# EnricoMiccoli/nodal

Hardware: AMD Instinct MI355X
Metric: circuits_per_sec (higher is better)
Workload: dtype f64; 1 GPU; cfg3: grid(1000) 1e6 nodes, sparse CSR path; n=999999, nnz=4995995, parallelism=one GPU

## Files before the change

nodal_amd/csrc/sagg.hip:

```cpp
#include <hip/hip_ext.h>

#include <atomic>
#include <type_traits>

#include "group.h"

int grounded_flags(nodal_ctx *h, uint8_t *flags_dev);

namespace {

using grp::TB;
constexpr int PW = 4;
constexpr int ACAP = 64;
constexpr int RCAP = 96;
constexpr int RCAP_SMALL = 512;
constexpr int RCAP_SMALL_ROWS = 16384;
inline int rcap_for(int64_t nc) { return nc <= RCAP_SMALL_ROWS ? RCAP_SMALL : RCAP; }
constexpr int W0_MAX = 32;
constexpr int COARSEST = 64;
constexpr int MAX_LEVELS = 12;
constexpr int MIS_ROUNDS = 6;
constexpr int TAIL_MAX_N = 1024;
constexpr int TAIL_LEVELS = 6;
constexpr int TAIL_LDS_BUDGET = 150 * 1024;
// ... 72 lines not shown
    int nlev;
    TailLevelDesc lv[TAIL_LEVELS];
    const double *inv;
    int nu;
    int image_bytes;
    int lds_bytes;
    int skip;
    int slots;
    long long *stamps;
};

struct SHierarchy {
    std::vector<SLevel *> pool;
    int nlev = 0;
    int tail = -1;
    bool ready = false;
    bool kcycle = true;
    bool kfrozen = false;
    int kslot = -1, kcount = 0, ksamples = 0;
    int klevels = 1;
    int nu[3] = {2, 1, 2};
    bool dense_coarsest = true;
    DevBuf tail_stamps, tail_image, apcol, apval, aplen, bstat;
    DevBuf mvec;
    hipEvent_t ev_copy = nullptr;
    hipStream_t aux = nullptr;
    hipEvent_t ev_fork = nullptr, ev_join = nullptr, ev_flags = nullptr;
    bool aux_pending = false;
    bool aux_tried = false;
    bool want_flags = false;
    int flags_levels = 0;
    DevBuf stats, coarse_inv, mis_t, mis_m, mis_flag, mis_id, agg1, keys, rstart, cursor, lists;
    TailDesc td;
    uint64_t *host_stats = nullptr;
    bool sym_valid = false;
    uint64_t sym_epoch = 0;
    int64_t sym_n = 0, sym_nnz = 0;
    bool sym_general = false, sym_check = false;
    int32_t sym_floating = 0;
    hipGraph_t it_graph = nullptr;
    hipGraphExec_t it_exec = nullptr;
    uint64_t it_key = 0;
    bool refreshed = false;
    int last_iters = 0;
    int hint_iters = 0;
    int64_t hint_n = 0, hint_nnz = 0;
// ... 5 lines not shown
        return pool[l];
    }
    void drop_graph() {
        if (it_exec) (void)hipGraphExecDestroy(it_exec);
        if (it_graph) (void)hipGraphDestroy(it_graph);
        it_exec = nullptr;
        it_graph = nullptr;
        it_key = 0;
    }
    ~SHierarchy() {
        drop_graph();
        if (ev_copy) (void)hipEventDestroy(ev_copy);
        if (ev_fork) (void)hipEventDestroy(ev_fork);
        if (ev_join) (void)hipEventDestroy(ev_join);
        if (ev_flags) (void)hipEventDestroy(ev_flags);
        if (aux) (void)hipStreamDestroy(aux);
        for (SLevel *l : pool) {
            DevBuf *b[] = {&l->acol, &l->aval, &l->alen, &l->dinv, &l->agg, &l->pcol, &l->pval, &l->rcol,
                           &l->rval, &l->rlen, &l->vec, &l->part, &l->gflag, &l->avalf, &l->pvalf, &l->rvalf, &l->adcol};
            for (DevBuf *x : b) x->release();
            delete l;
        }
        tail_image.release();
        mvec.release();
        tail_stamps.release();
        bstat.release();
        apcol.release();
        apval.release();
        aplen.release();
        DevBuf *b[] = {&stats, &coarse_inv, &mis_t, &mis_m, &mis_flag, &mis_id, &agg1, &keys, &rstart, &cursor, &lists};
        for (DevBuf *x : b) x->release();
        if (host_stats) (void)hipHostFree(host_stats);
    }
};


constexpr int BSTAT_MAX = 65536;
__global__ __launch_bounds__(1024) void reduce_bstat(int nblocks, const uint32_t *__restrict__ bstat,
                                                     unsigned long long *__restrict__ stats, int slot_max,
                                                     int slot_sum) {
    __shared__ unsigned int s_max;
    __shared__ unsigned long long s_sum;
    if (threadIdx.x == 0) { s_max = 0; s_sum = 0; }
    __syncthreads();
    unsigned int m = 0;
    unsigned long long t = 0;
// ... 1088 lines not shown
        NODAL_HIP_TRY(h, hipEventRecord(H->ev_join, H->aux));
        if (H->want_flags && H->flags_levels == l) {
            if (l == 0) NODAL_TRY(grounded_flags(h, L->gflag.as<uint8_t>()));
            NODAL_HIP_TRY(h, hipMemsetAsync(C->gflag.p, 0, ((size_t)C->n + 63) & ~(size_t)63, st));
            flags_up<<<grid_for(n), TB, 0, st>>>(n, L->agg.as<int32_t>(), L->gflag.as<uint8_t>(), C->gflag.as<uint8_t>());
            NODAL_HIP_TRY(h, hipGetLastError());
            NODAL_HIP_TRY(h, hipEventRecord(H->ev_flags, H->aux));
            H->flags_levels = l + 1;
        }
        h->stream = main_st;
        st = main_st;
    }
    NODAL_TRY(galerkin_product<false>(h, H, l, forked ? H->ev_join : nullptr, forked ? 2 : 0));
    if (forked && H->flags_levels != l + 1) H->aux_pending = false;
    return NODAL_OK;
}

const void *tail_kernel(int slots) {
    return slots <= 8 ? reinterpret_cast<const void *>(k_tail<8>)
                      : slots <= 16 ? reinterpret_cast<const void *>(k_tail<16>)
                                    : reinterpret_cast<const void *>(k_tail<32>);
}

int build_tail(nodal_ctx *h, SHierarchy *H, const unsigned long long *hs) {
    H->tail = -1;
    const int last = H->nlev - 1;
    auto up16 = [](int x) { return (x + 15) & ~15; };
    for (int t = 1; t <= last; ++t) {
        if (H->pool[t]->n > TAIL_MAX_N || last - t + 1 > TAIL_LEVELS) continue;
        TailDesc d;
        memset(&d, 0, sizeof d);
        d.nlev = last - t + 1;
        d.nu = getenv("NODAL_SA_TAIL_NU") ? atoi(getenv("NODAL_SA_TAIL_NU")) : 3;
        if (d.nu < 1) d.nu = 1;
        int off = 0;
        for (int k = 0; k < d.nlev; ++k) {
            const SLevel *L = H->pool[t + k];
            TailLevelDesc &q = d.lv[k];
            q.n = (int)L->n; q.nc = (int)L->nc; q.ld = (int)L->ld; q.rld = (int)L->rld; q.width = L->maxlen;
            q.acol = L->acol.as<int32_t>(); q.aval = L->aval.as<double>();
            q.dinv = L->dinv.as<double>(); q.alen = L->alen.as<int32_t>();
            q.pcol = L->pcol.as<int32_t>(); q.pval = L->pval.as<double>();
            q.rcol = L->rcol.as<int32_t>(); q.rval = L->rval.as<double>(); q.rlen = L->rlen.as<int32_t>();
            if (k == d.nlev - 1) {
                q.o_aval = off; off = up16(off + (H->dense_coarsest ? q.n * q.n : q.n) * 8);
                continue;
            }
            const int maxr = (int)hs[(size_t)(t + k) * ST_COUNT + ST_MAXR];
// ... 14 lines not shown
            q.o_B = off; off = up16(off + q.n * 8);
            q.o_X = off; off = up16(off + q.n * 8);
            if (k == d.nlev - 1) continue;
            q.o_Y = off; off = up16(off + q.n * 8);
            q.o_R = off; off = up16(off + q.n * 8);
        }
        d.inv = H->dense_coarsest ? H->coarse_inv.as<double>() : nullptr;
        d.skip = d.nlev > 1 ? d.lv[0].o_dinv : 0;
        d.lds_bytes = off - d.skip;
        if (getenv("NODAL_TAIL_PROBE")) {
            NODAL_HIP_TRY(h, H->tail_stamps.reserve(64 * sizeof(long long)));
            d.stamps = H->tail_stamps.as<long long>();
        }
        if (d.lds_bytes > TAIL_LDS_BUDGET) continue;
        d.slots = d.nlev > 1 ? (d.lv[0].width + d.lv[0].lpr - 1) / d.lv[0].lpr : 1;
        if (d.slots > 32) continue;
        {
            static std::atomic<bool> lds_allowed[64][3];
            const int dev = h->device >= 0 && h->device < 64 ? h->device : 0;
            const int which = d.slots <= 8 ? 0 : (d.slots <= 16 ? 1 : 2);
            if (!lds_allowed[dev][which].load(std::memory_order_acquire)) {
                NODAL_HIP_TRY(h, hipFuncSetAttribute(tail_kernel(d.slots), hipFuncAttributeMaxDynamicSharedMemorySize,
                                                     TAIL_LDS_BUDGET));
                lds_allowed[dev][which].store(true, std::memory_order_release);
            }
        }
        NODAL_HIP_TRY(h, H->tail_image.reserve((size_t)d.image_bytes + 256));
        k_tail_pack<<<1, 1024, 0, h->stream>>>(d, H->tail_image.as<char>());
        NODAL_HIP_TRY(h, hipGetLastError());
        H->td = d;
        H->tail = t;
        break;
    }
    return NODAL_OK;
}

int sagg_refresh(nodal_ctx *h, SHierarchy *H, const int32_t *indptr0, const int32_t *indices0, const double *data0,
                 bool general, bool *ok) {
    *ok = false;
    hipStream_t st = h->stream;
    unsigned long long *dstats = H->stats.as<unsigned long long>();
    unsigned long long *hs = reinterpret_cast<unsigned long long *>(H->host_stats);
    NODAL_HIP_TRY(h, hipMemsetAsync(dstats, 0, (size_t)MAX_LEVELS * ST_COUNT * 8, st));
    SLevel *L0 = H->pool[0];
    const int64_t n0 = L0->n;
    {
        const unsigned gr = grid_for(n0);
        static const double spread = getenv("NODAL_SA_SPREAD") ? atof(getenv("NODAL_SA_SPREAD")) : 16.0;
        static const double share = getenv("NODAL_SA_SHARE") ? atof(getenv("NODAL_SA_SHARE")) : 0.9;
        row_stats<<<gr, TB, 0, st>>>(n0, indptr0, indices0, data0, share, spread, general, dstats, H->bstat.as<uint32_t>());
        reduce_bstat<<<1, 1024, 0, st>>>((int)gr, H->bstat.as<uint32_t>(), dstats, ST_MAXLEN, ST_GRADED);
    }
    csr_to_ell<<<grid_for(n0), TB, 0, st>>>(n0, L0->ld, indptr0, indices0, data0, L0->acol.as<int32_t>(),
                                           L0->aval.as<double>(), L0->avalf.as<float>(),
// ... 9 lines not shown
        const bool forked = H->aux != nullptr && nodal_extra_streams_ok(h) &&
                            !(getenv("NODAL_SA_FORK") && atoi(getenv("NODAL_SA_FORK")) == 0);
        hipStream_t rst = st;
        if (forked) {
            NODAL_HIP_TRY(h, hipEventRecord(H->ev_fork, st));
            NODAL_HIP_TRY(h, hipStreamWaitEvent(H->aux, H->ev_fork, 0));
            H->aux_pending = true;
            NODAL_TRY(galerkin_product<true>(h, H, l, nullptr, 1));
            rst = H->aux;
        }
        r_refresh<<<grid_for(C->n * 8), TB, 0, rst>>>(C->n, L->rld, L->rlen.as<int32_t>(), L->rcol.as<int32_t>(), L->ld,
                                                     L->pcol.as<int32_t>(), L->pval.as<double>(), L->rval.as<double>(),
                                                     L->rvalf.as<float>());
        NODAL_HIP_TRY(h, hipGetLastError());
        if (forked) NODAL_HIP_TRY(h, hipEventRecord(H->ev_join, H->aux));
        NODAL_TRY(galerkin_product<true>(h, H, l, forked ? H->ev_join : nullptr, forked ? 2 : 0));
        if (forked) H->aux_pending = false;
    }
    const int last = H->nlev - 1;
    if (H->dense_coarsest)
        coarsest_inverse<<<1, 256, 0, st>>>(H->pool[last]->A(), H->coarse_inv.as<double>(), dstats + (size_t)last * ST_COUNT);
    if (H->tail >= 0) k_tail_pack<<<1, 1024, 0, st>>>(H->td, H->tail_image.as<char>());
    NODAL_HIP_TRY(h, hipGetLastError());
    NODAL_HIP_TRY(h, hipMemcpyAsync(hs, dstats, (size_t)MAX_LEVELS * ST_COUNT * 8, hipMemcpyDeviceToHost, st));
    NODAL_WAIT_STREAM(h, st);
    const int64_t bar = n0 / 100 < 32 ? (n0 / 100 > 0 ? n0 / 100 : 1) : 32;
    if (hs[ST_BADDIAG] || (int64_t)hs[ST_GRADED] >= bar) return NODAL_OK;
    for (int k = 1; k < H->nlev; ++k)
        if (hs[(size_t)k * ST_COUNT + ST_BADDIAG] || hs[(size_t)k * ST_COUNT + ST_OVERFLOW]) return NODAL_OK;
    *ok = true;
    return NODAL_OK;
}

}

void sagg_destroy(nodal_ctx *h) {
    delete static_cast<SHierarchy *>(h->sagg);
    h->sagg = nullptr;
}

static int sagg_setup_csr_body(nodal_ctx *h, int64_t n0, int64_t nnz0, const int32_t *indptr0, const int32_t *indices0,
                               const double *data0, bool general, bool check_floating, bool *accepted, int32_t *floating);

int sagg_setup_csr(nodal_ctx *h, int64_t n0, int64_t nnz0, const int32_t *indptr0, const int32_t *indices0,
                   const double *data0, bool general, bool check_floating, bool *accepted, int32_t *floating) {
    const int s = sagg_setup_csr_body(h, n0, nnz0, indptr0, indices0, data0, general, check_floating, accepted, floating);
// ... 192 lines not shown
    *accepted = true;
    H->sym_valid = true;
    H->sym_epoch = h->struct_epoch;
    H->sym_n = n0;
    H->sym_nnz = nnz0;
    H->sym_general = general;
    H->sym_check = check_floating;
    H->sym_floating = *floating;
    memcpy(H->sym_stats, hs, sizeof H->sym_stats);
    return NODAL_OK;
}

int sagg_setup(nodal_ctx *h, bool *accepted, int32_t *floating) {
    return sagg_setup_csr(h, h->n, h->nnz, h->indptr.as<int32_t>(), h->indices.as<int32_t>(), h->data.as<double>(),
                          false, true, accepted, floating);
}

namespace {

int last_level(nodal_ctx *h, SHierarchy *H, int l, const double *b, double *out) {
    hipStream_t st = h->stream;
    SLevel *L = H->pool[l];
    const int64_t n = L->n;
    if (l == H->tail) {
        if (H->td.slots <= 8) k_tail<8><<<1, 1024, (size_t)H->td.lds_bytes, st>>>(H->td, H->tail_image.as<char>(), b, out, 1);
        else if (H->td.slots <= 16) k_tail<16><<<1, 1024, (size_t)H->td.lds_bytes, st>>>(H->td, H->tail_image.as<char>(), b, out, 1);
        else k_tail<32><<<1, 1024, (size_t)H->td.lds_bytes, st>>>(H->td, H->tail_image.as<char>(), b, out, 1);
    } else {
        k_coarsest<<<grid_for(n), TB, 0, st>>>(n, H->dense_coarsest ? H->coarse_inv.as<double>() : nullptr,
                                               L->dinv.as<double>(), b, out);
    }
    NODAL_HIP_TRY(h, hipGetLastError());
    return NODAL_OK;
}

void kcycle_schedule(SHierarchy *H, int it) {
    static const bool on = !(getenv("NODAL_SA_KFREEZE") && atoi(getenv("NODAL_SA_KFREEZE")) == 0);
    H->kfrozen = false;
    H->kslot = -1;
    if (!on || it < 0) return;
    if (it == 0) H->ksamples = 0;
    const bool adaptive = it < 4 || (it & 3) == 0;
    if (!adaptive && H->ksamples > 0) {
        H->kfrozen = true;
    } else if (it >= 2) {
        H->kslot = H->ksamples % 3;
        ++H->ksamples;
        H->kcount = H->ksamples < 3 ? H->ksamples : 3;
    }
}

template <typename TBV, typename TOUT>
int cycle(nodal_ctx *h, SHierarchy *H, int l, const TBV *b, const cyc_t *x0, TOUT *out, const SolveBufs *sb) {
    hipStream_t st = h->stream;
// ... 255 lines not shown
            return NODAL_OK;
        }
        f_direction<<<sb.g0, TB, 0, st>>>(sb.z, sb.p, sb.part_rz, sb.part_zap, sb.part_rr, sb.g0, sb.sc, it & 1, n);
        const unsigned tb0 = H->pool[0]->wfix ? TB : TB * LPR_RAGGED;
        if (timed) {
            SAGG_DISPATCH_W(H->pool[0]->wfix, (hipExtLaunchKernelGGL((f_spmv<W>), dim3(sb.g0), dim3(tb0), 0, st, e0, e1, 0,
                                                                     A0, (const double *)sb.p, sb.Ap, sb.part_pap,
                                                                     (const double *)sb.sc, it & 1)));
        } else {
            SAGG_DISPATCH_W(H->pool[0]->wfix, (f_spmv<W><<<sb.g0, tb0, 0, st>>>(A0, sb.p, sb.Ap, sb.part_pap, sb.sc, it & 1)));
        }
        f_update<<<sb.g0, TB, 0, st>>>(x, sb.r, sb.p, sb.Ap, sb.part_pap, sb.g0, dinv0, sb.x0, sb.part_rr, sb.sc, it & 1, n);
        NODAL_HIP_TRY(h, hipGetLastError());
        return NODAL_OK;
    };
    static const bool graphs = getenv("NODAL_SA_GRAPH") && atoi(getenv("NODAL_SA_GRAPH")) != 0;
    if (graphs && (H->refreshed || !do_setup)) {
        uint64_t key = 1469598103934665603ull;
        auto mix = [&](uint64_t v) { key = (key ^ v) * 1099511628211ull; };
        mix((uint64_t)(uintptr_t)base); mix((uint64_t)(uintptr_t)x); mix((uint64_t)n); mix((uint64_t)sb.g0);
        mix((uint64_t)H->nlev); mix((uint64_t)(H->tail + 1)); mix((uint64_t)H->kcycle); mix((uint64_t)H->klevels);
        mix((uint64_t)(H->nu[0] * 100 + H->nu[1] * 10 + H->nu[2])); mix((uint64_t)H->td.lds_bytes);
        mix((uint64_t)(uintptr_t)H->tail_image.p); mix((uint64_t)(uintptr_t)H->coarse_inv.p);
        for (int k = 0; k < H->nlev; ++k) {
            const SLevel *L = H->pool[k];
            const void *ps[] = {L->acol.p, L->aval.p, L->avalf.p, L->alen.p, L->dinv.p, L->pcol.p, L->pvalf.p,
                                L->rcol.p, L->rvalf.p, L->rlen.p, L->vec.p, L->part.p};
            for (const void *q : ps) mix((uint64_t)(uintptr_t)q);
            mix((uint64_t)L->n); mix((uint64_t)L->ld); mix((uint64_t)L->wfix); mix((uint64_t)L->rld);
        }
        if (H->it_exec && H->it_key != key) H->drop_graph();
        if (!H->it_exec) {
            hipGraph_t g = nullptr;
            hipGraphExec_t ex = nullptr;
            if (hipStreamBeginCapture(st, hipStreamCaptureModeThreadLocal) == hipSuccess) {
                int cs = iteration(0, false);
                if (cs == NODAL_OK) cs = iteration(1, false);
                const hipError_t ce = hipStreamEndCapture(st, &g);
                if (cs == NODAL_OK && ce == hipSuccess && g && hipGraphInstantiate(&ex, g, nullptr, nullptr, 0) == hipSuccess) {
                    H->it_graph = g;
                    H->it_exec = ex;
                    H->it_key = key;
                } else {
                    if (g) (void)hipGraphDestroy(g);
                    (void)hipGetLastError();
                }
// ... 54 lines not shown
            const double target = tol * tol * hs[F_BB];
            const double rr_ref = rr_prev > 0.0 ? rr_prev : hs[F_BB];
            const int64_t it_ref = rr_prev > 0.0 ? it_prev : 0;
            if (hs[F_RR] > 0.0 && hs[F_RR] < rr_ref && enqueued > it_ref) {
                const double rate = log(hs[F_RR] / rr_ref) / (double)(enqueued - it_ref);
                static const double look = getenv("NODAL_FCG_LOOK") ? atof(getenv("NODAL_FCG_LOOK")) : 0.75;
                next = (int)floor(look * log(target / hs[F_RR]) / rate);
            }
            if (next > enqueued) next = (int)enqueued;
            batch = next < 1 ? 1 : (next > 32 ? 32 : next);
            rr_prev = hs[F_RR];
            it_prev = enqueued;
        }
    }
    const int64_t its = status == 1 ? (int64_t)hs[F_ITERS] : enqueued;
    *iters = (int32_t)its;
    *resid = hs[F_BB] > 0 ? sqrt(hs[F_RR] / hs[F_BB]) : 0.0;
    const SLevel *L0 = H->pool[0];
    h->kern_alg = 12.0 * (double)L0->nnz + 4.0 * (double)n + 16.0 * (double)n;
    if (fuse_dir) h->kern_alg += 12.0 * (double)n;
    if (trace)
        fprintf(stderr, "[sagg] %d iterations (%lld enqueued, %d polls), relative residual %.2e, status %d\n", *iters,
                (long long)enqueued, polls, *resid, status);
    if (trace && H->tail >= 0 && H->td.stamps) {
        long long ts[64];
        if (hipMemcpy(ts, H->td.stamps, sizeof ts, hipMemcpyDeviceToHost) == hipSuccess) {
            fprintf(stderr, "[sagg] tail phases (us):");
            for (int k = 1; k < (int)ts[63] && k < 63; ++k) fprintf(stderr, " %.2f", (double)(ts[k] - ts[k - 1]) * 0.01);
            fprintf(stderr, "  total %.2f, image %d B, lds %d B\n", (double)(ts[ts[63] - 1] - ts[0]) * 0.01,
                    H->td.image_bytes, H->td.lds_bytes);
            for (int k = 0; k < H->td.nlev; ++k)
                fprintf(stderr, "[sagg]   tail level %d: n %d width %d lpr %d nq %d\n", k, H->td.lv[k].n,
                        H->td.lv[k].width, H->td.lv[k].lpr, H->td.lv[k].nq);
        }
    }
    if (status != 1) {
        H->last_iters = 0;
        return -1;
    }
    H->last_iters = (int)its;
    H->hint_iters = (int)its;
    H->hint_n = n;
    H->hint_nnz = H->pool[0]->nnz;
    *info = 0;
    return NODAL_OK;
}

// ... 2 lines not shown
```

nodal_amd/csrc/sagg_cycle.h:

```cpp
#pragma once

namespace {

constexpr int LPR_RAGGED = 1;
template <int W> struct RowLanes { static constexpr int value = W == 0 ? LPR_RAGGED : 1; };

template <class VT, class XF>
__device__ __forceinline__ double ell_row_lanes(const Ell &A, const VT *__restrict__ val, int64_t i, int sub, XF xf) {
    constexpr int Q = 8;
    const int32_t len = A.len[i];
    double acc = 0.0;
    for (int32_t s0 = sub; s0 < len; s0 += LPR_RAGGED * Q) {
        int32_t c[Q];
        double v[Q];
        if (A.dcol) {
#pragma unroll
            for (int q = 0; q < Q; ++q) {
                const bool ok = s0 + q * LPR_RAGGED < len;
                const int64_t at = (int64_t)(ok ? s0 + q * LPR_RAGGED : s0) * A.ld + i;
                c[q] = (int32_t)i + (int32_t)A.dcol[at];
                const VT loaded = val[at];
                v[q] = ok ? (double)loaded : 0.0;
            }
        } else {
// ... 423 lines not shown
        copy_u16(u16(L.o_pcol), L.pcol, L.n, L.ld, PW);
        copy_f64(f64(L.o_rval), L.rval, L.nc * RL, (int64_t)L.rld * RL, L.nq);
        copy_u16(u16(L.o_rcol), L.rcol, L.nc * RL, (int64_t)L.rld * RL, L.nq);
    }
    const TailLevelDesc &L = d.lv[last];
    if (d.inv) copy_f64(f64(L.o_aval), d.inv, L.n * L.n, L.n * L.n, 1);
    else copy_f64(f64(L.o_aval), L.dinv, L.n, L.n, 1);
}

template <int SLOTS>
__device__ __forceinline__ double reg_row(const double (&v)[SLOTS], const uint32_t (&c)[SLOTS / 2], int lpr,
                                          const double *x) {
    double s0 = 0.0, s1 = 0.0;
#pragma unroll
    for (int j = 0; j < SLOTS; j += 2) {
        s0 = fma(v[j], x[c[j / 2] & 0xffffu], s0);
        s1 = fma(v[j + 1], x[c[j / 2] >> 16], s1);
    }
    double s = s0 + s1;
    for (int off = lpr >> 1; off > 0; off >>= 1) s += __shfl_xor(s, off, 64);
    return s;
}

template <int SLOTS>
__global__ __launch_bounds__(1024) void k_tail(TailDesc d, const char *__restrict__ image,
                                               const double *__restrict__ rc, double *__restrict__ out, int vs) {
    extern __shared__ __attribute__((aligned(16))) char smem[];
    const int tid = threadIdx.x;
    const int voff = vs > 1 ? (int)blockIdx.x : 0;
    const int last = d.nlev - 1;
    const int TAIL_NU = d.nu;
    auto f64 = [&](int off) { return reinterpret_cast<double *>(smem + (off - d.skip)); };
    auto u16 = [&](int off) { return reinterpret_cast<uint16_t *>(smem + (off - d.skip)); };
    int stamp_no = 0;
    auto stamp = [&]() {
        if (d.stamps && tid == 0) d.stamps[stamp_no] = wall_clock64();
        ++stamp_no;
    };
    stamp();
    double v0[SLOTS];
    uint32_t c0[SLOTS / 2];
    {
        const TailLevelDesc &L = d.lv[0];
        const double *aval = reinterpret_cast<const double *>(image + L.o_aval);
        const uint16_t *acol = reinterpret_cast<const uint16_t *>(image + L.o_acol);
        const int lpr = L.lpr, sub = tid & (lpr - 1), i = tid / lpr, ii = i < L.n ? i : L.n - 1;
        const bool row = last > 0 && i < L.n;
#pragma unroll
        for (int j = 0; j < SLOTS; j += 2) {
            const int ta = sub + j * lpr, tb = ta + lpr;
            const bool ha = row && ta < L.width, hb = row && tb < L.width;
            const int ea = ha ? ta * L.n + ii : 0, eb = hb ? tb * L.n + ii : 0;
            const double va = aval[ea], vb = aval[eb];
            const uint32_t ca = acol[ea], cb = acol[eb];
            v0[j] = ha ? va : 0.0;
            v0[j + 1] = hb ? vb : 0.0;
            c0[j / 2] = (ha ? ca : 0u) | ((hb ? cb : 0u) << 16);
        }
    }
    {
        constexpr int FLY = (TAIL_LDS_BUDGET / 16 + 1023) / 1024;
        const int4 *src = reinterpret_cast<const int4 *>(image + d.skip);
        int4 *dst = reinterpret_cast<int4 *>(smem);
        const int pieces = (d.image_bytes - d.skip) / 16;
        int4 v[FLY];
#pragma unroll
        for (int u = 0; u < FLY; ++u) v[u] = src[tid + u * 1024 < pieces ? tid + u * 1024 : 0];
#pragma unroll
        for (int u = 0; u < FLY; ++u)
            if (tid + u * 1024 < pieces) dst[tid + u * 1024] = v[u];
    }
    for (int i = tid; i < d.lv[0].n; i += 1024) f64(d.lv[0].o_B)[i] = rc[(int64_t)i * vs + voff];
    __syncthreads();
    stamp();
    for (int k = 0; k < last; ++k) {
        const TailLevelDesc &L = d.lv[k];
        const double *aval = f64(L.o_aval), *dinv = f64(L.o_dinv), *B = f64(L.o_B);
        const uint16_t *acol = u16(L.o_acol);
        double *X = f64(L.o_X), *Y = f64(L.o_Y), *R = f64(L.o_R);
        const int lpr = L.lpr, sub = tid & (lpr - 1), rows = 1024 / lpr;
        for (int i = tid; i < L.n; i += 1024) X[i] = OMEGA * dinv[i] * B[i];
        __syncthreads();
        for (int sweep = 1; sweep < TAIL_NU; ++sweep) {
            for (int i0 = 0; i0 < L.n; i0 += rows) {
                const int i = i0 + tid / lpr, ii = i < L.n ? i : L.n - 1;
                const double ax = k == 0 ? reg_row<SLOTS>(v0, c0, lpr, X)
                                         : lds_row(aval, acol, L.n, L.width, ii, sub, lpr, X);
                if (i < L.n && sub == 0) Y[i] = fma(OMEGA * dinv[i], B[i] - ax, X[i]);
            }
            __syncthreads();
            double *t = X; X = Y; Y = t;
        }
        for (int i0 = 0; i0 < L.n; i0 += rows) {
            const int i = i0 + tid / lpr, ii = i < L.n ? i : L.n - 1;
            const double ax = k == 0 ? reg_row<SLOTS>(v0, c0, lpr, X)
                                     : lds_row(aval, acol, L.n, L.width, ii, sub, lpr, X);
            if (i < L.n && sub == 0) R[i] = B[i] - ax;
        }
        __syncthreads();
        stamp();
        const double *rval = f64(L.o_rval);
        const uint16_t *rcol = u16(L.o_rcol);
        double *Bc = f64(d.lv[k + 1].o_B);
        for (int I0 = 0; I0 < L.nc; I0 += 1024 / RL) {
            const int I = I0 + tid / RL, r8 = tid & (RL - 1);
            double s = 0.0;
            if (I < L.nc) {
                double s1 = 0.0;
                const int e0 = I * RL + r8, step = L.nc * RL;
                int q = 0;
                for (; q + 3 < L.nq; q += 4) {
                    const int ea = e0 + q * step, eb = ea + step, ec = eb + step, ed = ec + step;
                    const double va = rval[ea], vb = rval[eb], vc = rval[ec], vd = rval[ed];
                    const int ca = rcol[ea], cb = rcol[eb], cc = rcol[ec], cd = rcol[ed];
                    s = fma(va, R[ca], s);
                    s1 = fma(vb, R[cb], s1);
                    s = fma(vc, R[cc], s);
                    s1 = fma(vd, R[cd], s1);
                }
                for (; q < L.nq; ++q) s = fma(rval[e0 + q * step], R[rcol[e0 + q * step]], s);
                s += s1;
            }
#pragma unroll
            for (int off = RL >> 1; off > 0; off >>= 1) s += __shfl_xor(s, off, 64);
            if (I < L.nc && r8 == 0) Bc[I] = s;
        }
        __syncthreads();
        stamp();
    }
    {
        const TailLevelDesc &L = d.lv[last];
        const double *inv = f64(L.o_aval), *B = f64(L.o_B);
        double *E = f64(L.o_X);
        for (int i = tid; i < L.n; i += 1024) {
            double s = 0.0;
            if (d.inv) {
                double s1 = 0.0, s2 = 0.0, s3 = 0.0;
                const double *row = inv + i * L.n;
                int j = 0;
                for (; j + 3 < L.n; j += 4) {
                    s = fma(row[j], B[j], s);
                    s1 = fma(row[j + 1], B[j + 1], s1);
                    s2 = fma(row[j + 2], B[j + 2], s2);
                    s3 = fma(row[j + 3], B[j + 3], s3);
                }
                for (; j < L.n; ++j) s = fma(row[j], B[j], s);
                s = (s + s1) + (s2 + s3);
            } else {
                s = inv[i] * B[i];
            }
            E[i] = s;
        }
        __syncthreads();
        stamp();
    }
    const double *Ec = f64(d.lv[last].o_X);
    for (int k = last - 1; k >= 0; --k) {
        const TailLevelDesc &L = d.lv[k];
        const double *aval = f64(L.o_aval), *dinv = f64(L.o_dinv), *B = f64(L.o_B), *pval = f64(L.o_pval);
        const uint16_t *acol = u16(L.o_acol), *pcol = u16(L.o_pcol);
        double *X = f64((TAIL_NU & 1) ? L.o_X : L.o_Y), *Y = f64((TAIL_NU & 1) ? L.o_Y : L.o_X);
        for (int i = tid; i < L.n; i += 1024) {
            double s = X[i];
#pragma unroll
            for (int q = 0; q < PW; ++q) s = fma(pval[q * L.n + i], Ec[pcol[q * L.n + i]], s);
            Y[i] = s;
        }
        __syncthreads();
        stamp();
        const int lpr = L.lpr, sub = tid & (lpr - 1), rows = 1024 / lpr;
        for (int sweep = 0; sweep < TAIL_NU; ++sweep) {
            for (int i0 = 0; i0 < L.n; i0 += rows) {
                const int i = i0 + tid / lpr, ii = i < L.n ? i : L.n - 1;
                const double ax = k == 0 ? reg_row<SLOTS>(v0, c0, lpr, Y)
                                         : lds_row(aval, acol, L.n, L.width, ii, sub, lpr, Y);
                if (i < L.n && sub == 0) X[i] = fma(OMEGA * dinv[i], B[i] - ax, Y[i]);
            }
            __syncthreads();
            double *t = X; X = Y; Y = t;
        }
        Ec = Y;
        stamp();
    }
    for (int i = tid; i < d.lv[0].n; i += 1024) out[(int64_t)i * vs + voff] = Ec[i];
    stamp();
    if (d.stamps && tid == 0) d.stamps[63] = stamp_no;
}

enum { F_RZ = 0, F_ALPHA = 2, F_CONV = 4, F_RR = 6, F_BB = 7, F_FLAG = 8, F_ITERS = 9, F_TOL2 = 10,
       F_ITNO = 12,
       F_COUNT = 16 };
constexpr int MAX_PARTIALS = 1024;

__global__ __launch_bounds__(TB) void f_init(const double *__restrict__ b, double *__restrict__ x,
                                             double *__restrict__ r, double *__restrict__ Ap,
                                             const double *__restrict__ dinv, cyc_t *__restrict__ x0,
                                             double *__restrict__ part_rr, int64_t n) {
    double srr = 0.0;
    for (int64_t i = (int64_t)xcd_block() * TB + threadIdx.x; i < n; i += (int64_t)gridDim.x * TB) {
        const double ri = b[i];
        x[i] = 0.0;
        r[i] = ri;
        x0[i] = (cyc_t)(OMEGA * dinv[i] * ri);
        Ap[i] = 0.0;
        srr = fma(ri, ri, srr);
    }
    srr = block_sum(srr);
    if (threadIdx.x == 0) part_rr[blockIdx.x] = srr;
}
// ... 190 lines not shown
```

nodal_amd/csrc/sagg_multi.h:

```cpp
#pragma once

namespace {

#ifndef NODAL_MK_SHIFT
#define NODAL_MK_SHIFT 4
#endif
constexpr int MK = 1 << NODAL_MK_SHIFT;
constexpr int MK_SHIFT = NODAL_MK_SHIFT;
constexpr int MSC = 32;
enum { M_SUM = 16, M_INC = 17 , M_RING = 4, M_FDONE = 21 };
constexpr int MPARTS = 1024;

template <int NQ>
__device__ __forceinline__ void column_partials(double (&a)[NQ], double *__restrict__ part, int cap) {
    __shared__ double ws[NQ][TB / 64][MK];
    const int lane = threadIdx.x & 63, wave = threadIdx.x >> 6;
#pragma unroll
    for (int q = 0; q < NQ; ++q) {
        double v = a[q];
#pragma unroll
        for (int off = MK; off < 64; off <<= 1) v += __shfl_xor(v, off, 64);
        if (lane < MK) ws[q][wave][lane] = v;
    }
    __syncthreads();
// ... 404 lines not shown
struct MLevel {
    double *vec = nullptr;
    double *part = nullptr;
    double *tot = nullptr;
    int64_t ld = 0;
    template <typename T> T *v(int which) const { return reinterpret_cast<T *>(vec + (int64_t)which * ld * MK); }
};
struct MBufs {
    MLevel lv[MAX_LEVELS];
    double *x, *r, *p, *Ap;
    cyc_t *z, *x0;
    double *part;
    double *tot;
    double *sc;
    int32_t *ia, *ib;
    int g0;
};
constexpr int MDOT = 1024;

int m_last_level(nodal_ctx *h, SHierarchy *H, int l, const double *b, double *out) {
    hipStream_t st = h->stream;
    SLevel *L = H->pool[l];
    const int64_t n = L->n;
    if (l == H->tail) {
        if (H->td.slots <= 8) k_tail<8><<<MK, 1024, (size_t)H->td.lds_bytes, st>>>(H->td, H->tail_image.as<char>(), b, out, MK);
        else if (H->td.slots <= 16) k_tail<16><<<MK, 1024, (size_t)H->td.lds_bytes, st>>>(H->td, H->tail_image.as<char>(), b, out, MK);
        else k_tail<32><<<MK, 1024, (size_t)H->td.lds_bytes, st>>>(H->td, H->tail_image.as<char>(), b, out, MK);
    } else {
        m_coarsest<<<mgrid(n), TB, 0, st>>>(n, H->dense_coarsest ? H->coarse_inv.as<double>() : nullptr,
                                            L->dinv.as<double>(), b, out);
    }
    NODAL_HIP_TRY(h, hipGetLastError());
    return NODAL_OK;
}

template <typename TBV>
int m_cycle(nodal_ctx *h, SHierarchy *H, const MBufs &M, int l, const TBV *b, const cyc_t *x0, cyc_t *out, bool outer) {
    hipStream_t st = h->stream;
    SLevel *L = H->pool[l];
    const int64_t n = L->n;
    SLevel *C = H->pool[l + 1];
    const int64_t nc = C->n;
    const Ell A = L->A();
    const bool f32 = L->avalf.p != nullptr;
    const double *dinv = L->dinv.as<double>();
    const MLevel &ML = M.lv[l], &MC = M.lv[l + 1];
    const cyc_t *x = x0;
    cyc_t *r = ML.v<cyc_t>(V_R), *xp = ML.v<cyc_t>(V_XP);
    const unsigned g = mgrid(n);
    const unsigned gp = outer ? (unsigned)M.g0 : mgrid(n);
    const int nu = H->nu[l < 2 ? l : 2];
    if (nu >= 2) {
        cyc_t *x1 = ML.v<cyc_t>(V_X1);
        SAGG_DISPATCH_W(L->wfix, (m_post<W, false, TBV><<<g, TB, 0, st>>>(A, dinv, b, x0, x1, nullptr, nullptr, 0, f32)));
// ... 228 lines not shown
```

Measured before the change: 147.8 circuits/s.

## Precompute tail multigrid cycle as dense operator and apply it by matvec

Since the tail V-cycle is a linear map on a small coarse level (n<=1024), it is formed once at setup as a dense n×n matrix by running the cycle on unit vectors, one column per block. The per-iteration coarse solve then becomes a parallel dense matvec across many blocks instead of a single 1024-thread block walking several levels with many barriers. Setup cost rises (n cycle evaluations, O(n^2) storage), and results differ by rounding only. An env var can disable it, and an optional self-check compares the two paths.

```diff
diff --git a/nodal_amd/csrc/sagg.hip b/nodal_amd/csrc/sagg.hip
--- a/nodal_amd/csrc/sagg.hip
+++ b/nodal_amd/csrc/sagg.hip
@@ -118,6 +118,8 @@
     int nu[3] = {2, 1, 2};
     bool dense_coarsest = true;
     DevBuf tail_stamps, tail_image, apcol, apval, aplen, bstat;
+    DevBuf tail_op;
+    bool tail_dense = false;
     DevBuf mvec;
     hipEvent_t ev_copy = nullptr;
     hipStream_t aux = nullptr;
@@ -169,6 +171,7 @@
             delete l;
         }
         tail_image.release();
+        tail_op.release();
         mvec.release();
         tail_stamps.release();
         bstat.release();
@@ -1303,8 +1306,106 @@
                                     : reinterpret_cast<const void *>(k_tail<32>);
 }
 
+const void *tail_op_kernel(int slots) {
+    return slots <= 8 ? reinterpret_cast<const void *>(k_tail_pack_op<8>)
+                      : slots <= 16 ? reinterpret_cast<const void *>(k_tail_pack_op<16>)
+                                    : reinterpret_cast<const void *>(k_tail_pack_op<32>);
+}
+
+int tail_walk(nodal_ctx *h, SHierarchy *H, const double *b, double *out, int nv) {
+    const TailDesc &d = H->td;
+    const char *img = H->tail_image.as<char>();
+    if (d.slots <= 8) k_tail<8><<<nv, 1024, (size_t)d.lds_bytes, h->stream>>>(d, img, b, out, nv);
+    else if (d.slots <= 16) k_tail<16><<<nv, 1024, (size_t)d.lds_bytes, h->stream>>>(d, img, b, out, nv);
+    else k_tail<32><<<nv, 1024, (size_t)d.lds_bytes, h->stream>>>(d, img, b, out, nv);
+    NODAL_HIP_TRY(h, hipGetLastError());
+    return NODAL_OK;
+}
+
+template <int NV>
+int tail_apply(nodal_ctx *h, SHierarchy *H, const double *b, double *out) {
+    const int n = H->td.lv[0].n;
+    const double *T = H->tail_op.as<double>();
+    const unsigned gr = (unsigned)((n + 3) / 4);
+    if (n <= 256) k_tail_apply<4, NV><<<gr, 256, 0, h->stream>>>(n, T, b, out);
+    else if (n <= 512) k_tail_apply<8, NV><<<gr, 256, 0, h->stream>>>(n, T, b, out);
+    else k_tail_apply<16, NV><<<gr, 256, 0, h->stream>>>(n, T, b, out);
+    NODAL_HIP_TRY(h, hipGetLastError());
+    return NODAL_OK;
+}
+
+int tail_self_check(nodal_ctx *h, SHierarchy *H) {
+    const int n = H->td.lv[0].n;
+    std::vector<double> b((size_t)n), yc((size_t)n), yd((size_t)n), T((size_t)n * n);
+    uint64_t seed = 0x9e3779b97f4a7c15ull;
+    for (int i = 0; i < n; ++i) {
+        uint64_t z = (seed += 0x9e3779b97f4a7c15ull);
+        z = (z ^ (z >> 30)) * 0xbf58476d1ce4e5b9ull;
+        z = (z ^ (z >> 27)) * 0x94d049bb133111ebull;
+        z ^= z >> 31;
+        b[i] = (double)(z >> 11) * (1.0 / 4503599627370496.0) - 1.0;
+    }
+    DevBuf v;
+    hipError_t e = v.reserve((size_t)3 * n * 8);
+    double *db = v.as<double>(), *dc = db + n, *dd = dc + n;
+    int rc = NODAL_OK;
+    if (e == hipSuccess) e = hipMemcpyAsync(db, b.data(), (size_t)n * 8, hipMemcpyHostToDevice, h->stream);
+    if (e == hipSuccess) rc = tail_walk(h, H, db, dc, 1);
+    if (e == hipSuccess && rc == NODAL_OK) rc = tail_apply<1>(h, H, db, dd);
+    if (e == hipSuccess && rc == NODAL_OK) e = hipStreamSynchronize(h->stream);
+    if (e == hipSuccess) e = hipMemcpy(yc.data(), dc, (size_t)n * 8, hipMemcpyDeviceToHost);
+    if (e == hipSuccess) e = hipMemcpy(yd.data(), dd, (size_t)n * 8, hipMemcpyDeviceToHost);
+    if (e == hipSuccess) e = hipMemcpy(T.data(), H->tail_op.p, (size_t)n * n * 8, hipMemcpyDeviceToHost);
+    v.release();
+    if (rc != NODAL_OK) return rc;
+    NODAL_HIP_TRY(h, e);
+    double d = 0.0, dp = 0.0;
+    for (int i = 0; i < n; ++i) {
+        long double y = 0.0L, a = 0.0L;
+        for (int j = 0; j < n; ++j) {
+            y += (long double)T[(size_t)i * n + j] * b[j];
+            a += fabsl((long double)T[(size_t)i * n + j] * b[j]);
+        }
+        const double den = (double)a;
+        const double q = fabs(yd[i] - yc[i]) / den, qp = (double)(fabsl((long double)yd[i] - y) / a);
+        d = !(q <= d) ? q : d;
+        dp = !(qp <= dp) ? qp : dp;
+    }
+    fprintf(stderr, "[sagg] tail check: n_t %d, dense operator against the cycle d = %.3e (product alone %.3e)\n", n, d, dp);
+    return NODAL_OK;
+}
+
+int form_tail_op(nodal_ctx *h, SHierarchy *H) {
+    static const bool on = !(getenv("NODAL_SA_TAIL_DENSE") && atoi(getenv("NODAL_SA_TAIL_DENSE")) == 0);
+    H->tail_dense = false;
+    if (!on || H->tail < 0) return NODAL_OK;
+    const TailDesc &d = H->td;
+    const int n = d.lv[0].n;
+    static std::atomic<int> cus[64];
+    const int dev = h->device >= 0 && h->device < 64 ? h->device : 0;
+    int ncu = cus[dev].load(std::memory_order_acquire);
+    if (ncu == 0) {
+        NODAL_HIP_TRY(h, hipDeviceGetAttribute(&ncu, hipDeviceAttributeMultiprocessorCount, h->device >= 0 ? h->device : 0));
+        if (ncu < 1) ncu = 1;
+        cus[dev].store(ncu, std::memory_order_release);
+    }
+    NODAL_HIP_TRY(h, H->tail_op.reserve((size_t)n * n * 8 + 64));
+    const unsigned gr = (unsigned)(n < ncu ? n : ncu);
+    double *T = H->tail_op.as<double>();
+    const char *img = H->tail_image.as<char>();
+    if (d.slots <= 8) k_tail_pack_op<8><<<gr, 1024, (size_t)d.lds_bytes, h->stream>>>(d, img, T);
+    else if (d.slots <= 16) k_tail_pack_op<16><<<gr, 1024, (size_t)d.lds_bytes, h->stream>>>(d, img, T);
+    else k_tail_pack_op<32><<<gr, 1024, (size_t)d.lds_bytes, h->stream>>>(d, img, T);
+    NODAL_HIP_TRY(h, hipGetLastError());
+    H->tail_dense = true;
+    static const bool check = getenv("NODAL_TRACE") && getenv("NODAL_SA_TAIL_CHECK") && atoi(getenv("NODAL_SA_TAIL_CHECK")) != 0;
+    if (check) NODAL_TRY(tail_self_check(h, H));
+    return NODAL_OK;
+}
+
 int build_tail(nodal_ctx *h, SHierarchy *H, const unsigned long long *hs) {
     H->tail = -1;
+    H->tail_dense = false;
     const int last = H->nlev - 1;
     auto up16 = [](int x) { return (x + 15) & ~15; };
     for (int t = 1; t <= last; ++t) {
@@ -1365,6 +1466,8 @@
             if (!lds_allowed[dev][which].load(std::memory_order_acquire)) {
                 NODAL_HIP_TRY(h, hipFuncSetAttribute(tail_kernel(d.slots), hipFuncAttributeMaxDynamicSharedMemorySize,
                                                      TAIL_LDS_BUDGET));
+                NODAL_HIP_TRY(h, hipFuncSetAttribute(tail_op_kernel(d.slots), hipFuncAttributeMaxDynamicSharedMemorySize,
+                                                     TAIL_LDS_BUDGET));
                 lds_allowed[dev][which].store(true, std::memory_order_release);
             }
         }
@@ -1373,6 +1476,7 @@
         NODAL_HIP_TRY(h, hipGetLastError());
         H->td = d;
         H->tail = t;
+        NODAL_TRY(form_tail_op(h, H));
         break;
     }
     return NODAL_OK;
@@ -1428,6 +1532,7 @@
         coarsest_inverse<<<1, 256, 0, st>>>(H->pool[last]->A(), H->coarse_inv.as<double>(), dstats + (size_t)last * ST_COUNT);
     if (H->tail >= 0) k_tail_pack<<<1, 1024, 0, st>>>(H->td, H->tail_image.as<char>());
     NODAL_HIP_TRY(h, hipGetLastError());
+    NODAL_TRY(form_tail_op(h, H));
     NODAL_HIP_TRY(h, hipMemcpyAsync(hs, dstats, (size_t)MAX_LEVELS * ST_COUNT * 8, hipMemcpyDeviceToHost, st));
     NODAL_WAIT_STREAM(h, st);
     const int64_t bar = n0 / 100 < 32 ? (n0 / 100 > 0 ? n0 / 100 : 1) : 32;
@@ -1666,14 +1771,9 @@
     hipStream_t st = h->stream;
     SLevel *L = H->pool[l];
     const int64_t n = L->n;
-    if (l == H->tail) {
-        if (H->td.slots <= 8) k_tail<8><<<1, 1024, (size_t)H->td.lds_bytes, st>>>(H->td, H->tail_image.as<char>(), b, out, 1);
-        else if (H->td.slots <= 16) k_tail<16><<<1, 1024, (size_t)H->td.lds_bytes, st>>>(H->td, H->tail_image.as<char>(), b, out, 1);
-        else k_tail<32><<<1, 1024, (size_t)H->td.lds_bytes, st>>>(H->td, H->tail_image.as<char>(), b, out, 1);
-    } else {
-        k_coarsest<<<grid_for(n), TB, 0, st>>>(n, H->dense_coarsest ? H->coarse_inv.as<double>() : nullptr,
-                                               L->dinv.as<double>(), b, out);
-    }
+    if (l == H->tail) return H->tail_dense ? tail_apply<1>(h, H, b, out) : tail_walk(h, H, b, out, 1);
+    k_coarsest<<<grid_for(n), TB, 0, st>>>(n, H->dense_coarsest ? H->coarse_inv.as<double>() : nullptr,
+                                           L->dinv.as<double>(), b, out);
     NODAL_HIP_TRY(h, hipGetLastError());
     return NODAL_OK;
 }
@@ -1975,6 +2075,7 @@
         mix((uint64_t)H->nlev); mix((uint64_t)(H->tail + 1)); mix((uint64_t)H->kcycle); mix((uint64_t)H->klevels);
         mix((uint64_t)(H->nu[0] * 100 + H->nu[1] * 10 + H->nu[2])); mix((uint64_t)H->td.lds_bytes);
         mix((uint64_t)(uintptr_t)H->tail_image.p); mix((uint64_t)(uintptr_t)H->coarse_inv.p);
+        mix((uint64_t)(uintptr_t)(H->tail_dense ? H->tail_op.p : nullptr));
         for (int k = 0; k < H->nlev; ++k) {
             const SLevel *L = H->pool[k];
             const void *ps[] = {L->acol.p, L->aval.p, L->avalf.p, L->alen.p, L->dinv.p, L->pcol.p, L->pvalf.p,
@@ -2075,7 +2176,7 @@
     if (trace)
         fprintf(stderr, "[sagg] %d iterations (%lld enqueued, %d polls), relative residual %.2e, status %d\n", *iters,
                 (long long)enqueued, polls, *resid, status);
-    if (trace && H->tail >= 0 && H->td.stamps) {
+    if (trace && H->tail >= 0 && H->td.stamps && !H->tail_dense) {
         long long ts[64];
         if (hipMemcpy(ts, H->td.stamps, sizeof ts, hipMemcpyDeviceToHost) == hipSuccess) {
             fprintf(stderr, "[sagg] tail phases (us):");
diff --git a/nodal_amd/csrc/sagg_cycle.h b/nodal_amd/csrc/sagg_cycle.h
--- a/nodal_amd/csrc/sagg_cycle.h
+++ b/nodal_amd/csrc/sagg_cycle.h
@@ -469,19 +469,17 @@
     return s;
 }
 
-template <int SLOTS>
-__global__ __launch_bounds__(1024) void k_tail(TailDesc d, const char *__restrict__ image,
-                                               const double *__restrict__ rc, double *__restrict__ out, int vs) {
-    extern __shared__ __attribute__((aligned(16))) char smem[];
+template <int SLOTS, bool UNIT>
+__device__ __forceinline__ void tail_cycle(const TailDesc &d, char *smem, const char *__restrict__ image,
+                                           const double *__restrict__ rc, double *__restrict__ out, int vs, int voff) {
     const int tid = threadIdx.x;
-    const int voff = vs > 1 ? (int)blockIdx.x : 0;
     const int last = d.nlev - 1;
     const int TAIL_NU = d.nu;
     auto f64 = [&](int off) { return reinterpret_cast<double *>(smem + (off - d.skip)); };
     auto u16 = [&](int off) { return reinterpret_cast<uint16_t *>(smem + (off - d.skip)); };
     int stamp_no = 0;
     auto stamp = [&]() {
-        if (d.stamps && tid == 0) d.stamps[stamp_no] = wall_clock64();
+        if (!UNIT && d.stamps && tid == 0) d.stamps[stamp_no] = wall_clock64();
         ++stamp_no;
     };
     stamp();
@@ -517,121 +515,192 @@
         for (int u = 0; u < FLY; ++u)
             if (tid + u * 1024 < pieces) dst[tid + u * 1024] = v[u];
     }
-    for (int i = tid; i < d.lv[0].n; i += 1024) f64(d.lv[0].o_B)[i] = rc[(int64_t)i * vs + voff];
-    __syncthreads();
-    stamp();
-    for (int k = 0; k < last; ++k) {
-        const TailLevelDesc &L = d.lv[k];
-        const double *aval = f64(L.o_aval), *dinv = f64(L.o_dinv), *B = f64(L.o_B);
-        const uint16_t *acol = u16(L.o_acol);
-        double *X = f64(L.o_X), *Y = f64(L.o_Y), *R = f64(L.o_R);
-        const int lpr = L.lpr, sub = tid & (lpr - 1), rows = 1024 / lpr;
-        for (int i = tid; i < L.n; i += 1024) X[i] = OMEGA * dinv[i] * B[i];
+    for (;;) {
+        for (int i = tid; i < d.lv[0].n; i += 1024)
+            f64(d.lv[0].o_B)[i] = UNIT ? (i == voff ? 1.0 : 0.0) : rc[(int64_t)i * vs + voff];
         __syncthreads();
-        for (int sweep = 1; sweep < TAIL_NU; ++sweep) {
+        stamp();
+        for (int k = 0; k < last; ++k) {
+            const TailLevelDesc &L = d.lv[k];
+            const double *aval = f64(L.o_aval), *dinv = f64(L.o_dinv), *B = f64(L.o_B);
+            const uint16_t *acol = u16(L.o_acol);
+            double *X = f64(L.o_X), *Y = f64(L.o_Y), *R = f64(L.o_R);
+            const int lpr = L.lpr, sub = tid & (lpr - 1), rows = 1024 / lpr;
+            for (int i = tid; i < L.n; i += 1024) X[i] = OMEGA * dinv[i] * B[i];
+            __syncthreads();
+            for (int sweep = 1; sweep < TAIL_NU; ++sweep) {
+                for (int i0 = 0; i0 < L.n; i0 += rows) {
+                    const int i = i0 + tid / lpr, ii = i < L.n ? i : L.n - 1;
+                    const double ax = k == 0 ? reg_row<SLOTS>(v0, c0, lpr, X)
+                                             : lds_row(aval, acol, L.n, L.width, ii, sub, lpr, X);
+                    if (i < L.n && sub == 0) Y[i] = fma(OMEGA * dinv[i], B[i] - ax, X[i]);
+                }
+                __syncthreads();
+                double *t = X; X = Y; Y = t;
+            }
             for (int i0 = 0; i0 < L.n; i0 += rows) {
                 const int i = i0 + tid / lpr, ii = i < L.n ? i : L.n - 1;
                 const double ax = k == 0 ? reg_row<SLOTS>(v0, c0, lpr, X)
                                          : lds_row(aval, acol, L.n, L.width, ii, sub, lpr, X);
-                if (i < L.n && sub == 0) Y[i] = fma(OMEGA * dinv[i], B[i] - ax, X[i]);
+                if (i < L.n && sub == 0) R[i] = B[i] - ax;
             }
             __syncthreads();
-            double *t = X; X = Y; Y = t;
-        }
-        for (int i0 = 0; i0 < L.n; i0 += rows) {
-            const int i = i0 + tid / lpr, ii = i < L.n ? i : L.n - 1;
-            const double ax = k == 0 ? reg_row<SLOTS>(v0, c0, lpr, X)
-                                     : lds_row(aval, acol, L.n, L.width, ii, sub, lpr, X);
-            if (i < L.n && sub == 0) R[i] = B[i] - ax;
-        }
+            stamp();
+            const double *rval = f64(L.o_rval);
+            const uint16_t *rcol = u16(L.o_rcol);
+            double *Bc = f64(d.lv[k + 1].o_B);
+            for (int I0 = 0; I0 < L.nc; I0 += 1024 / RL) {
+                const int I = I0 + tid / RL, r8 = tid & (RL - 1);
+                double s = 0.0;
+                if (I < L.nc) {
+                    double s1 = 0.0;
+                    const int e0 = I * RL + r8, step = L.nc * RL;
+                    int q = 0;
+                    for (; q + 3 < L.nq; q += 4) {
+                        const int ea = e0 + q * step, eb = ea + step, ec = eb + step, ed = ec + step;
+                        const double va = rval[ea], vb = rval[eb], vc = rval[ec], vd = rval[ed];
+                        const int ca = rcol[ea], cb = rcol[eb], cc = rcol[ec], cd = rcol[ed];
+                        s = fma(va, R[ca], s);
+                        s1 = fma(vb, R[cb], s1);
+                        s = fma(vc, R[cc], s);
+                        s1 = fma(vd, R[cd], s1);
+                    }
+                    for (; q < L.nq; ++q) s = fma(rval[e0 + q * step], R[rcol[e0 + q * step]], s);
+                    s += s1;
+                }
+#pragma unroll
+                for (int off = RL >> 1; off > 0; off >>= 1) s += __shfl_xor(s, off, 64);
+                if (I < L.nc && r8 == 0) Bc[I] = s;
+            }
+            __syncthreads();
+            stamp();
+        }
+        {
+            const TailLevelDesc &L = d.lv[last];
+            const double *inv = f64(L.o_aval), *B = f64(L.o_B);
+            double *E = f64(L.o_X);
+            for (int i = tid; i < L.n; i += 1024) {
+                double s = 0.0;
+                if (d.inv) {
+                    double s1 = 0.0, s2 = 0.0, s3 = 0.0;
+                    const double *row = inv + i * L.n;
+                    int j = 0;
+                    for (; j + 3 < L.n; j += 4) {
+                        s = fma(row[j], B[j], s);
+                        s1 = fma(row[j + 1], B[j + 1], s1);
+                        s2 = fma(row[j + 2], B[j + 2], s2);
+                        s3 = fma(row[j + 3], B[j + 3], s3);
+                    }
+                    for (; j < L.n; ++j) s = fma(row[j], B[j], s);
+                    s = (s + s1) + (s2 + s3);
+                } else {
+                    s = inv[i] * B[i];
+                }
+                E[i] = s;
+            }
+            __syncthreads();
+            stamp();
+        }
+        const double *Ec = f64(d.lv[last].o_X);
+        for (int k = last - 1; k >= 0; --k) {
+            const TailLevelDesc &L = d.lv[k];
+            const double *aval = f64(L.o_aval), *dinv = f64(L.o_dinv), *B = f64(L.o_B), *pval = f64(L.o_pval);
+            const uint16_t *acol = u16(L.o_acol), *pcol = u16(L.o_pcol);
+            double *X = f64((TAIL_NU & 1) ? L.o_X : L.o_Y), *Y = f64((TAIL_NU & 1) ? L.o_Y : L.o_X);
+            for (int i = tid; i < L.n; i += 1024) {
+                double s = X[i];
+#pragma unroll
+                for (int q = 0; q < PW; ++q) s = fma(pval[q * L.n + i], Ec[pcol[q * L.n + i]], s);
+                Y[i] = s;
+            }
+            __syncthreads();
+            stamp();
+            const int lpr = L.lpr, sub = tid & (lpr - 1), rows = 1024 / lpr;
+            for (int sweep = 0; sweep < TAIL_NU; ++sweep) {
+                for (int i0 = 0; i0 < L.n; i0 += rows) {
+                    const int i = i0 + tid / lpr, ii = i < L.n ? i : L.n - 1;
+                    const double ax = k == 0 ? reg_row<SLOTS>(v0, c0, lpr, Y)
+                                             : lds_row(aval, acol, L.n, L.width, ii, sub, lpr, Y);
+                    if (i < L.n && sub == 0) X[i] = fma(OMEGA * dinv[i], B[i] - ax, Y[i]);
+                }
+                __syncthreads();
+                double *t = X; X = Y; Y = t;
+            }
+            Ec = Y;
+            stamp();
+        }
+        for (int i = tid; i < d.lv[0].n; i += 1024) out[(int64_t)i * vs + voff] = Ec[i];
+        stamp();
+        voff += (int)gridDim.x;
+        if (!UNIT || voff >= d.lv[0].n) break;
         __syncthreads();
-        stamp();
-        const double *rval = f64(L.o_rval);
-        const uint16_t *rcol = u16(L.o_rcol);
-        double *Bc = f64(d.lv[k + 1].o_B);
-        for (int I0 = 0; I0 < L.nc; I0 += 1024 / RL) {
-            const int I = I0 + tid / RL, r8 = tid & (RL - 1);
-            double s = 0.0;
-            if (I < L.nc) {
-                double s1 = 0.0;
-                const int e0 = I * RL + r8, step = L.nc * RL;
-                int q = 0;
-                for (; q + 3 < L.nq; q += 4) {
-                    const int ea = e0 + q * step, eb = ea + step, ec = eb + step, ed = ec + step;
-                    const double va = rval[ea], vb = rval[eb], vc = rval[ec], vd = rval[ed];
-                    const int ca = rcol[ea], cb = rcol[eb], cc = rcol[ec], cd = rcol[ed];
-                    s = fma(va, R[ca], s);
-                    s1 = fma(vb, R[cb], s1);
-                    s = fma(vc, R[cc], s);
-                    s1 = fma(vd, R[cd], s1);
-                }
-                for (; q < L.nq; ++q) s = fma(rval[e0 + q * step], R[rcol[e0 + q * step]], s);
-                s += s1;
-            }
-#pragma unroll
-            for (int off = RL >> 1; off > 0; off >>= 1) s += __shfl_xor(s, off, 64);
-            if (I < L.nc && r8 == 0) Bc[I] = s;
-        }
-        __syncthreads();
-        stamp();
-    }
-    {
-        const TailLevelDesc &L = d.lv[last];
-        const double *inv = f64(L.o_aval), *B = f64(L.o_B);
-        double *E = f64(L.o_X);
-        for (int i = tid; i < L.n; i += 1024) {
-            double s = 0.0;
-            if (d.inv) {
-                double s1 = 0.0, s2 = 0.0, s3 = 0.0;
-                const double *row = inv + i * L.n;
-                int j = 0;
-                for (; j + 3 < L.n; j += 4) {
-                    s = fma(row[j], B[j], s);
-                    s1 = fma(row[j + 1], B[j + 1], s1);
-                    s2 = fma(row[j + 2], B[j + 2], s2);
-                    s3 = fma(row[j + 3], B[j + 3], s3);
-                }
-                for (; j < L.n; ++j) s = fma(row[j], B[j], s);
-                s = (s + s1) + (s2 + s3);
-            } else {
-                s = inv[i] * B[i];
-            }
-            E[i] = s;
-        }
-        __syncthreads();
-        stamp();
-    }
-    const double *Ec = f64(d.lv[last].o_X);
-    for (int k = last - 1; k >= 0; --k) {
-        const TailLevelDesc &L = d.lv[k];
-        const double *aval = f64(L.o_aval), *dinv = f64(L.o_dinv), *B = f64(L.o_B), *pval = f64(L.o_pval);
-        const uint16_t *acol = u16(L.o_acol), *pcol = u16(L.o_pcol);
-        double *X = f64((TAIL_NU & 1) ? L.o_X : L.o_Y), *Y = f64((TAIL_NU & 1) ? L.o_Y : L.o_X);
-        for (int i = tid; i < L.n; i += 1024) {
-            double s = X[i];
-#pragma unroll
-            for (int q = 0; q < PW; ++q) s = fma(pval[q * L.n + i], Ec[pcol[q * L.n + i]], s);
-            Y[i] = s;
-        }
-        __syncthreads();
-        stamp();
-        const int lpr = L.lpr, sub = tid & (lpr - 1), rows = 1024 / lpr;
-        for (int sweep = 0; sweep < TAIL_NU; ++sweep) {
-            for (int i0 = 0; i0 < L.n; i0 += rows) {
-                const int i = i0 + tid / lpr, ii = i < L.n ? i : L.n - 1;
-                const double ax = k == 0 ? reg_row<SLOTS>(v0, c0, lpr, Y)
-                                         : lds_row(aval, acol, L.n, L.width, ii, sub, lpr, Y);
-                if (i < L.n && sub == 0) X[i] = fma(OMEGA * dinv[i], B[i] - ax, Y[i]);
-            }
-            __syncthreads();
-            double *t = X; X = Y; Y = t;
-        }
-        Ec = Y;
-        stamp();
-    }
-    for (int i = tid; i < d.lv[0].n; i += 1024) out[(int64_t)i * vs + voff] = Ec[i];
-    stamp();
-    if (d.stamps && tid == 0) d.stamps[63] = stamp_no;
+    }
+    if (!UNIT && d.stamps && tid == 0) d.stamps[63] = stamp_no;
+}
+
+template <int SLOTS>
+__global__ __launch_bounds__(1024) void k_tail(TailDesc d, const char *__restrict__ image,
+                                               const double *__restrict__ rc, double *__restrict__ out, int vs) {
+    extern __shared__ __attribute__((aligned(16))) char smem[];
+    tail_cycle<SLOTS, false>(d, smem, image, rc, out, vs, vs > 1 ? (int)blockIdx.x : 0);
+}
+
+template <int SLOTS>
+__global__ __launch_bounds__(1024) void k_tail_pack_op(TailDesc d, const char *__restrict__ image,
+                                                       double *__restrict__ T) {
+    extern __shared__ __attribute__((aligned(16))) char smem[];
+    tail_cycle<SLOTS, true>(d, smem, image, nullptr, T, d.lv[0].n, (int)blockIdx.x);
+}
+
+template <int CH, int NV>
+__global__ __launch_bounds__(256) void k_tail_apply(int n, const double *__restrict__ T,
+                                                    const double *__restrict__ rc, double *__restrict__ out) {
+    const int lane = threadIdx.x & 63;
+    const int i = (int)blockIdx.x * 4 + (threadIdx.x >> 6);
+    if (i >= n) return;
+    const double *row = T + (int64_t)i * n;
+    double t[CH];
+#pragma unroll
+    for (int u = 0; u < CH; ++u) {
+        const int j = lane + 64 * u;
+        t[u] = row[j < n ? j : 0];
+    }
+    if constexpr (NV == 1) {
+        double r[CH];
+#pragma unroll
+        for (int u = 0; u < CH; ++u) {
+            const int j = lane + 64 * u;
+            r[u] = rc[j < n ? j : 0];
+        }
+        double s0 = 0.0, s1 = 0.0;
+#pragma unroll
+        for (int u = 0; u < CH; u += 2) {
+            if (lane + 64 * u < n && t[u] != 0.0) s0 = fma(t[u], r[u], s0);
+            if (lane + 64 * (u + 1) < n && t[u + 1] != 0.0) s1 = fma(t[u + 1], r[u + 1], s1);
+        }
+        const double s = wave_sum(s0 + s1);
+        if (lane == 0) out[i] = s;
+    } else {
+        double s[NV];
+#pragma unroll
+        for (int c = 0; c < NV; ++c) s[c] = 0.0;
+#pragma unroll
+        for (int u = 0; u < CH; ++u) {
+            const int j = lane + 64 * u;
+            const double *rj = rc + (int64_t)(j < n ? j : 0) * NV;
+            const bool use = j < n && t[u] != 0.0;
+#pragma unroll
+            for (int c = 0; c < NV; ++c) {
+                const double v = rj[c];
+                if (use) s[c] = fma(t[u], v, s[c]);
+            }
+        }
+#pragma unroll
+        for (int c = 0; c < NV; ++c) {
+            const double v = wave_sum(s[c]);
+            if (lane == 0) out[(int64_t)i * NV + c] = v;
+        }
+    }
 }
 
 enum { F_RZ = 0, F_ALPHA = 2, F_CONV = 4, F_RR = 6, F_BB = 7, F_FLAG = 8, F_ITERS = 9, F_TOL2 = 10,
diff --git a/nodal_amd/csrc/sagg_multi.h b/nodal_amd/csrc/sagg_multi.h
--- a/nodal_amd/csrc/sagg_multi.h
+++ b/nodal_amd/csrc/sagg_multi.h
@@ -450,14 +450,10 @@
     hipStream_t st = h->stream;
     SLevel *L = H->pool[l];
     const int64_t n = L->n;
-    if (l == H->tail) {
-        if (H->td.slots <= 8) k_tail<8><<<MK, 1024, (size_t)H->td.lds_bytes, st>>>(H->td, H->tail_image.as<char>(), b, out, MK);
-        else if (H->td.slots <= 16) k_tail<16><<<MK, 1024, (size_t)H->td.lds_bytes, st>>>(H->td, H->tail_image.as<char>(), b, out, MK);
-        else k_tail<32><<<MK, 1024, (size_t)H->td.lds_bytes, st>>>(H->td, H->tail_image.as<char>(), b, out, MK);
-    } else {
-        m_coarsest<<<mgrid(n), TB, 0, st>>>(n, H->dense_coarsest ? H->coarse_inv.as<double>() : nullptr,
-                                            L->dinv.as<double>(), b, out);
-    }
+    if (l == H->tail)
+        return H->tail_dense ? tail_apply<MK>(h, H, b, out) : tail_walk(h, H, b, out, MK);
+    m_coarsest<<<mgrid(n), TB, 0, st>>>(n, H->dense_coarsest ? H->coarse_inv.as<double>() : nullptr,
+                                        L->dinv.as<double>(), b, out);
     NODAL_HIP_TRY(h, hipGetLastError());
     return NODAL_OK;
 }
```

Result: faster. 159.3 circuits/s, median of 6 (+7.8%).
